# SADPR/1D-Burgers-Equation-ROMs

Hardware: AMD Instinct MI355X
Metric: batched Newton-steps/sec over mu-sweep (sample-Newton-steps/s, FOM N=1024) (higher is better)
Workload: dtype f64

## Files before the change

### 1d-burgers-equation-roms_amd/csrc/fom.hip

```cpp
#include <hip/hip_runtime.h>
#include <stdint.h>
#include <type_traits>

#include "../../include/burgers_hip.h"
#include "abi_common.hpp"
#include "fom_device.hpp"
#include "fom_wide.hpp"

namespace bg {
thread_local int tls_last_hip_error = 0;
}

namespace {

using namespace bg;

struct FomArgs {
    const double* x;
    const double* u0;
    const double* mu1;
    const double* mu2;
    double* hist;
    int32_t* iters;
    int32_t* flags;
    double dt, E, tol2;
    int N, B, nsteps, max_it, supg;
    double* errs;
};

constexpr int WAVES_PER_WG = 4;

template <int R>
__device__ __forceinline__ void load_rows(const double* __restrict__ src, int N, int row0, bool full,
                                          double (&u)[R], double pad = 0.0)
{
#pragma unroll
    for (int j = 0; j < R; ++j) u[j] = (full || row0 + j < N) ? src[row0 + j] : pad;
}

template <int R>
__device__ __forceinline__ void store_rows(double* __restrict__ dst, int N, int row0, bool full,
                                           const double (&u)[R])
{
#pragma unroll
    for (int j = 0; j < R; ++j)
        if (full || row0 + j < N) dst[row0 + j] = u[j];
}

template <int R, bool FULL, bool UNI, bool TRACE, bool PARK, class Topo>
__device__ __forceinline__ void fom_sample(const FomArgs& a, Topo& tp, int s, WidePark<PARK ? R : 1>* park)
{
    static_assert(UNI || !PARK, "only the uniform assembly reads g and hfs through accessors");
    const int N = a.N, t = tp.g, row0 = t * R;
    const double h = (a.x[N - 1] - a.x[0]) / (double)(N - 1);
    const MeshConst c = make_mesh_const(h, a.dt, a.E, a.supg);
    const double mu1 = a.mu1[s], mu2 = a.mu2[s];

    double hfs[PARK ? 1 : R], fdt[R], u[R], g[PARK ? 1 : R];
    ElemGeom<UNI ? 0 : R> gm;
    if constexpr (PARK) {
        double hf[R];
        forcing_setup<R>(a.x, N, row0, mu2, c.h, a.dt, hf, fdt);
#pragma unroll
        for (int j = 0; j < R; ++j) park->hfs[j][t] = hf[j];
    } else if constexpr (UNI) {
        forcing_setup<R>(a.x, N, row0, mu2, c.h, a.dt, hfs, fdt);
    } else {
        geom_setup<R>(a.x, N, row0, a.dt, a.E, gm);
        forcing_setup_general<R>(a.x, N, row0, mu2, a.dt, hfs, fdt);
    }
    auto g_put = [&](int j, double v) { if constexpr (PARK) park->g[j][t] = v; else g[j] = v; };
    auto g_at = [&](int j) { if constexpr (PARK) return park->g[j][t]; else return g[j]; };
    auto hf_at = [&](int j) { if constexpr (PARK) return park->hfs[j][t]; else return hfs[j]; };

    double* hist = a.hist + (size_t)s * (size_t)(a.nsteps + 1) * (size_t)N;
    load_rows<R>(a.u0 + (size_t)s * N, N, row0, FULL, u);
    store_rows<R>(hist, N, row0, FULL, u);

    int flags = 0;
    for (int step = 0; step < a.nsteps; ++step) {
        if constexpr (UNI) mass_rhs<R, FULL>(tp, c, N, u, fdt, g_put);
        else mass_rhs_general<R>(tp, gm, N, u, fdt, g);
        int k = 0;
        bool more;
        do {
            double lo[R], di[R], up[R], rhs[R];
            if constexpr (UNI) assemble<R, FULL>(tp, c, N, mu1, u, g_at, hf_at, lo, di, up, rhs);
            else assemble_general<R>(tp, gm, a.dt, c.kap, N, mu1, u, g, hfs, lo, di, up, rhs);
            tp.template solve<R>(lo, di, up, rhs);
            double nd = 0.0, nu = 0.0;
#pragma unroll
            for (int j = 0; j < R; ++j) {
                u[j] += rhs[j];
                nd = __builtin_fma(rhs[j], rhs[j], nd);
                nu = __builtin_fma(u[j], u[j], nu);
            }
            tp.sum2(nd, nu, nd, nu);
            if constexpr (TRACE) {
                if (tp.first()) a.errs[((size_t)s * a.nsteps + step) * a.max_it + k] = sqrt(nd) / sqrt(nu);
            }
            ++k;
            more = (nd > a.tol2 * nu) && (k < a.max_it);
            flags |= uniform_nonfinite(nd, nu) ? BG_FLAG_NONFINITE : 0;
        } while (more);
        if (k >= a.max_it) flags |= BG_FLAG_HIT_CAP;
        store_rows<R>(hist + (size_t)(step + 1) * N, N, row0, FULL, u);
        if (tp.first()) a.iters[(size_t)s * a.nsteps + step] = k;
    }
    if (tp.first()) a.flags[s] = flags;
}

struct AsmArgs {
    const double *x, *uk, *un, *mu1, *mu2;
    double *lo, *di, *up, *rhs;
    double dt, E;
    int N, B, supg;
};

template <int R, bool FULL, bool UNI, class Topo>
__device__ __forceinline__ void assemble_sample(const AsmArgs& a, Topo& tp, int s)
{
    const int N = a.N, row0 = tp.g * R;
    const double h = (a.x[N - 1] - a.x[0]) / (double)(N - 1);
    const MeshConst c = make_mesh_const(h, a.dt, a.E, a.supg);
    double hfs[R], fdt[R], u[R], un[R], g[R], lo[R], di[R], up[R], rhs[R];
    load_rows<R>(a.un + (size_t)s * N, N, row0, FULL, un);
    load_rows<R>(a.uk + (size_t)s * N, N, row0, FULL, u);
    if constexpr (UNI) {
        forcing_setup<R>(a.x, N, row0, a.mu2[s], c.h, a.dt, hfs, fdt);
        auto g_put = [&](int j, double v) { g[j] = v; };
        auto g_at = [&](int j) { return g[j]; };
        auto hf_at = [&](int j) { return hfs[j]; };
        mass_rhs<R, FULL>(tp, c, N, un, fdt, g_put);
        assemble<R, FULL>(tp, c, N, a.mu1[s], u, g_at, hf_at, lo, di, up, rhs);
    } else {
        ElemGeom<R> gm;
        geom_setup<R>(a.x, N, row0, a.dt, a.E, gm);
        forcing_setup_general<R>(a.x, N, row0, a.mu2[s], a.dt, hfs, fdt);
        mass_rhs_general<R>(tp, gm, N, un, fdt, g);
        assemble_general<R>(tp, gm, a.dt, c.kap, N, a.mu1[s], u, g, hfs, lo, di, up, rhs);
    }
    store_rows<R>(a.lo + (size_t)s * N, N, row0, FULL, lo);
    store_rows<R>(a.di + (size_t)s * N, N, row0, FULL, di);
    store_rows<R>(a.up + (size_t)s * N, N, row0, FULL, up);
    store_rows<R>(a.rhs + (size_t)s * N, N, row0, FULL, rhs);
}

struct SolveArgs {
    const double *lo, *di, *up, *rhs;
    double* sol;
    int N, B;
};

template <int R, class Topo>
__device__ __forceinline__ void solve_sample(const SolveArgs& a, Topo& tp, int s)
{
    const int N = a.N, row0 = tp.g * R;
    double lo[R], di[R], up[R], rhs[R];
    const size_t off = (size_t)s * N;
    load_rows<R>(a.lo + off, N, row0, false, lo);
    load_rows<R>(a.di + off, N, row0, false, di, 1.0);
    load_rows<R>(a.up + off, N, row0, false, up);
    load_rows<R>(a.rhs + off, N, row0, false, rhs);
    tp.template solve<R>(lo, di, up, rhs);
    store_rows<R>(a.sol + off, N, row0, false, rhs);
}

template <int R, bool FULL, bool UNI = true, bool TRACE = false>
__global__ __launch_bounds__(64 * WAVES_PER_WG, 1) void fom_fused_kernel(FomArgs a)
{
    const int s = blockIdx.x * WAVES_PER_WG + (int)(threadIdx.x >> 6);
    if (s >= a.B) return;
    WaveTopo tp{lane_id()};
    fom_sample<R, FULL, UNI, TRACE, false>(a, tp, s, nullptr);
}

template <int R, bool FULL, bool UNI = true>
__global__ __launch_bounds__(64 * WAVES_PER_WG, 1) void fom_assemble_kernel(AsmArgs a)
{
    const int s = blockIdx.x * WAVES_PER_WG + (int)(threadIdx.x >> 6);
    if (s >= a.B) return;
    WaveTopo tp{lane_id()};
    assemble_sample<R, FULL, UNI>(a, tp, s);
}

template <int R>
__global__ __launch_bounds__(64 * WAVES_PER_WG, 1) void tridiag_solve_kernel(SolveArgs a)
{
    const int s = blockIdx.x * WAVES_PER_WG + (int)(threadIdx.x >> 6);
    if (s >= a.B) return;
    WaveTopo tp{lane_id()};
    solve_sample<R>(a, tp, s);
}

template <int R, bool UNI>
__global__ __launch_bounds__(WIDE_THREADS, 1) void fom_wide_kernel(FomArgs a)
{
    constexpr bool PARK = UNI && R >= 32;
    __shared__ WideLds lds;
    __shared__ WidePark<PARK ? R : 1> park;
    wide_init(lds, threadIdx.x);
    WgTopo tp{lds, (int)threadIdx.x, 0};
    fom_sample<R, false, UNI, false, PARK>(a, tp, blockIdx.x, &park);
}

template <int R, bool UNI>
__global__ __launch_bounds__(WIDE_THREADS, 1) void fom_assemble_wide_kernel(AsmArgs a)
{
    __shared__ WideLds lds;
    wide_init(lds, threadIdx.x);
    WgTopo tp{lds, (int)threadIdx.x, 0};
    assemble_sample<R, false, UNI>(a, tp, blockIdx.x);
}

template <int R>
__global__ __launch_bounds__(WIDE_THREADS, 1) void tridiag_solve_wide_kernel(SolveArgs a)
{
    __shared__ WideLds lds;
    wide_init(lds, threadIdx.x);
    WgTopo tp{lds, (int)threadIdx.x, 0};
    solve_sample<R>(a, tp, blockIdx.x);
}

__global__ __launch_bounds__(256) void transpose_kernel(const double* __restrict__ in,
                                                        double* __restrict__ out, int nb, int rows, int cols)
{
    __shared__ double tile[32][33];
    const int c0 = blockIdx.x * 32, r0 = blockIdx.y * 32;
    const int tx = threadIdx.x & 31, ty = threadIdx.x >> 5;
    for (int b = blockIdx.z; b < nb; b += gridDim.z) {
        const size_t base = (size_t)b * rows * cols;
#pragma unroll
        for (int k = 0; k < 32; k += 8) {
            int r = r0 + ty + k, cc = c0 + tx;
            if (r < rows && cc < cols) tile[ty + k][tx] = in[base + (size_t)r * cols + cc];
        }
        __syncthreads();
#pragma unroll
        for (int k = 0; k < 32; k += 8) {
            int cc = c0 + ty + k, r = r0 + tx;
            if (r < rows && cc < cols) out[base + (size_t)cc * rows + r] = tile[tx][ty + k];
        }
        __syncthreads();
    }
}

constexpr int kWaveMaxN = 64 * 24, kWideMaxN = WIDE_THREADS * 32;

template <typename F>
int dispatch_wide(int N, F&& f)
{
    return dispatch_rows<WIDE_THREADS, 2, 4, 8, 12, 16, 24, 32>(N, f);
}

template <typename F>
int dispatch_r(int N, F&& f)
{
    return dispatch_rows<64, 1, 2, 3, 4, 5, 6, 8, 9, 10, 12, 16, 24>(N, f);
}

int fom_args(FomArgs& a, bool traced, int N, int B, int nsteps, const double* x, const double* u0, const double* mu1,
             const double* mu2, double dt, double E, double tol, int max_it, int supg, double* hist, int32_t* iters,
             int32_t* flags, double* errs)
{
    if (N < 2 || B < 0 || nsteps < 0 || max_it < 1 || !(dt > 0.0)) return BG_ERR_BAD_ARG;
    if (traced && N > kWaveMaxN) return BG_ERR_UNSUPPORTED_N;
    if (B == 0) return BG_OK;
    if (!x || !u0 || !mu1 || !mu2 || !hist || !flags || (traced && !errs) || (nsteps > 0 && !iters)) return BG_ERR_BAD_ARG;
    a.x = x; a.u0 = u0; a.mu1 = mu1; a.mu2 = mu2; a.hist = hist; a.iters = iters; a.flags = flags; a.errs = errs;
    a.dt = dt; a.E = E; a.tol2 = tol * tol;
    a.N = N; a.B = B; a.nsteps = nsteps; a.max_it = max_it; a.supg = supg & BG_OPT_SUPG;
    return BG_OK;
}

}

extern "C" {

int bg_abi_version(void) { return BG_ABI_VERSION; }

int bg_last_hip_error(void) { return bg::tls_last_hip_error; }

int bg_fom_max_n(void) { return kWideMaxN; }

const char* bg_strerror(int code)
{
    switch (code) {
        case BG_OK: return "ok";
        case BG_ERR_BAD_ARG: return "bad argument";
        case BG_ERR_UNSUPPORTED_N: return "N not supported by the fused kernels (2 <= N <= 8192)";
        case BG_ERR_NONUNIFORM: return "mesh is not uniform";
        case BG_ERR_LAUNCH: return "kernel launch failed (see bg_last_hip_error)";
        case BG_ERR_UNSUPPORTED_R: return "reduced dimension not supported";
        case BG_ERR_PROJECTION: return "unknown projection";
        case BG_ERR_WORKSPACE: return "workspace too small";
        default: return "unknown error";
    }
}

int bg_fom_run(int N, int B, int nsteps, const double* x, const double* u0, const double* mu1,
               const double* mu2, double dt, double E, double tol, int max_it, int supg, double* hist,
               int32_t* iters, int32_t* flags, void* stream)
{
    FomArgs a;
    const int err = fom_args(a, false, N, B, nsteps, x, u0, mu1, mu2, dt, E, tol, max_it, supg, hist, iters, flags, nullptr);
    if (err != BG_OK || B == 0) return err;
    const bool nonuniform = (supg & BG_OPT_NONUNIFORM) != 0;
    const dim3 grid((B + WAVES_PER_WG - 1) / WAVES_PER_WG), block(64 * WAVES_PER_WG);
    hipStream_t st = (hipStream_t)stream;
    const bool both = N <= kWaveMaxN && N > 64 && !nonuniform;
    const bool wide = N > kWaveMaxN || (both && (supg & BG_OPT_FOM_WIDE) && !(supg & BG_OPT_FOM_WAVE));
    if (wide)
        return dispatch_wide(N, [&](auto rc) {
            constexpr int R = decltype(rc)::value;
            if constexpr (R >= 8) {
                if (nonuniform) {
                    hipLaunchKernelGGL((fom_wide_kernel<R, false>), dim3(B), dim3(WIDE_THREADS), 0, st, a);
                    return check_launch();
                }
            }
            hipLaunchKernelGGL((fom_wide_kernel<R, true>), dim3(B), dim3(WIDE_THREADS), 0, st, a);
            return check_launch();
        });
    return dispatch_r(N, [&](auto rc) {
        constexpr int R = decltype(rc)::value;
        if (nonuniform)
            hipLaunchKernelGGL((fom_fused_kernel<R, false, false>), grid, block, 0, st, a);
        else if (N == 64 * R)
            hipLaunchKernelGGL((fom_fused_kernel<R, true>), grid, block, 0, st, a);
        else
            hipLaunchKernelGGL((fom_fused_kernel<R, false>), grid, block, 0, st, a);
        return check_launch();
    });
}

int bg_fom_run_traced(int N, int B, int nsteps, const double* x, const double* u0, const double* mu1, const double* mu2,
                      double dt, double E, double tol, int max_it, int supg, double* hist, int32_t* iters, int32_t* flags,
                      double* errs, void* stream)
{
    FomArgs a;
    const int err = fom_args(a, true, N, B, nsteps, x, u0, mu1, mu2, dt, E, tol, max_it, supg, hist, iters, flags, errs);
    if (err != BG_OK || B == 0) return err;
    const bool nonuniform = (supg & BG_OPT_NONUNIFORM) != 0;
    const dim3 grid((B + WAVES_PER_WG - 1) / WAVES_PER_WG), block(64 * WAVES_PER_WG);
    hipStream_t st = (hipStream_t)stream;
    return dispatch_r(N, [&](auto rc) {
        constexpr int R = decltype(rc)::value;
        if (nonuniform)
            hipLaunchKernelGGL((fom_fused_kernel<R, false, false, true>), grid, block, 0, st, a);
        else
            hipLaunchKernelGGL((fom_fused_kernel<R, false, true, true>), grid, block, 0, st, a);
        return check_launch();
    });
}

int bg_fom_assemble(int N, int B, const double* x, const double* uk, const double* un, const double* mu1,
                    const double* mu2, double dt, double E, int supg, double* lo, double* di, double* up,
                    double* rhs, void* stream)
{
    if (N < 2 || B < 0 || !(dt > 0.0)) return BG_ERR_BAD_ARG;
    if (B == 0) return BG_OK;
    if (!x || !uk || !un || !mu1 || !mu2 || !lo || !di || !up || !rhs) return BG_ERR_BAD_ARG;
    AsmArgs a;
    a.x = x; a.uk = uk; a.un = un; a.mu1 = mu1; a.mu2 = mu2; a.lo = lo; a.di = di; a.up = up; a.rhs = rhs;
    a.dt = dt; a.E = E; a.N = N; a.B = B; a.supg = supg & BG_OPT_SUPG;
    const bool nonuniform = (supg & BG_OPT_NONUNIFORM) != 0;
    const dim3 grid((B + WAVES_PER_WG - 1) / WAVES_PER_WG), block(64 * WAVES_PER_WG);
    hipStream_t st = (hipStream_t)stream;
    if (N > kWaveMaxN)
        return dispatch_wide(N, [&](auto rc) {
            constexpr int R = decltype(rc)::value;
            if (nonuniform)
                hipLaunchKernelGGL((fom_assemble_wide_kernel<R, false>), dim3(B), dim3(WIDE_THREADS), 0, st, a);
            else
                hipLaunchKernelGGL((fom_assemble_wide_kernel<R, true>), dim3(B), dim3(WIDE_THREADS), 0, st, a);
            return check_launch();
        });
    return dispatch_r(N, [&](auto rc) {
        constexpr int R = decltype(rc)::value;
        if (nonuniform)
            hipLaunchKernelGGL((fom_assemble_kernel<R, false, false>), grid, block, 0, st, a);
        else if (N == 64 * R)
            hipLaunchKernelGGL((fom_assemble_kernel<R, true>), grid, block, 0, st, a);
        else
            hipLaunchKernelGGL((fom_assemble_kernel<R, false>), grid, block, 0, st, a);
        return check_launch();
    });
}

int bg_tridiag_solve(int N, int B, const double* lo, const double* di, const double* up, const double* rhs,
                     double* sol, void* stream)
{
    if (N < 1 || B < 0) return BG_ERR_BAD_ARG;
    if (B == 0) return BG_OK;
    if (!lo || !di || !up || !rhs || !sol) return BG_ERR_BAD_ARG;
    SolveArgs a{lo, di, up, rhs, sol, N, B};
    const dim3 grid((B + WAVES_PER_WG - 1) / WAVES_PER_WG), block(64 * WAVES_PER_WG);
    hipStream_t st = (hipStream_t)stream;
    if (N > kWaveMaxN)
        return dispatch_wide(N, [&](auto rc) {
            constexpr int R = decltype(rc)::value;
            hipLaunchKernelGGL((tridiag_solve_wide_kernel<R>), dim3(B), dim3(WIDE_THREADS), 0, st, a);
            return check_launch();
        });
    return dispatch_r(N, [&](auto rc) {
        constexpr int R = decltype(rc)::value;
        hipLaunchKernelGGL((tridiag_solve_kernel<R>), grid, block, 0, st, a);
        return check_launch();
    });
}

int bg_transpose_batched(int B, int rows, int cols, const double* in, double* out, void* stream)
{
    if (B < 0 || rows < 0 || cols < 0) return BG_ERR_BAD_ARG;
    if (B == 0 || rows == 0 || cols == 0) return BG_OK;
    if (!in || !out) return BG_ERR_BAD_ARG;
    const dim3 grid((cols + 31) / 32, (rows + 31) / 32, B < 65535 ? B : 65535), block(256);
    hipLaunchKernelGGL(transpose_kernel, grid, block, 0, (hipStream_t)stream, in, out, B, rows, cols);
    return check_launch();
}

}
```

### 1d-burgers-equation-roms_amd/csrc/fom_device.hpp

```cpp
#pragma once
#include "wave_ops.hpp"

#ifndef BG_RCP
#define BG_RCP rcp1
#endif

#ifndef BG_PCR_EARLY_EXIT
#define BG_PCR_EARLY_EXIT 1
#endif

namespace bg {

constexpr double GP_A = 0.78867513459481287;
constexpr double GP_B = 0.21132486540518713;

struct MeshConst {
    double h;
    double aoff;
    double dd2;
    double dd1;
    double dt6;
    double kap;
    double h6;
};

__device__ __forceinline__ MeshConst make_mesh_const(double h, double dt, double E, int supg)
{
    MeshConst c;
    c.h = h;
    double eh = dt * E / h;
    c.aoff = h / 6.0 - eh;
    c.dd1 = h / 3.0 + eh;
    c.dd2 = 2.0 * c.dd1;
    c.dt6 = dt / 6.0;
    c.kap = supg ? 0.25 * dt : 0.0;
    c.h6 = h / 6.0;
    return c;
}

template <int R>
__device__ __forceinline__ void forcing_setup(const double* __restrict__ x, int N, int row0, double mu2,
                                              double h, double dt, double (&hfs)[R], double (&fdt)[R])
{
    double frPrev = 0.0;
    {
        int e = row0 - 1;
        if (e >= 0 && e < N - 1) {
            double xl = x[e], xr = x[e + 1];
            double f1 = 0.02 * exp(mu2 * (GP_A * xl + GP_B * xr));
            double f2 = 0.02 * exp(mu2 * (GP_B * xl + GP_A * xr));
            frPrev = (f1 * GP_B + f2 * GP_A) * (0.5 * h);
        }
    }
#pragma unroll
    for (int j = 0; j < R; ++j) {
        int e = row0 + j;
        double fl = 0.0, fr = 0.0, fs = 0.0;
        if (e < N - 1) {
            double xl = x[e], xr = x[e + 1];
            double f1 = 0.02 * exp(mu2 * (GP_A * xl + GP_B * xr));
            double f2 = 0.02 * exp(mu2 * (GP_B * xl + GP_A * xr));
            fl = (f1 * GP_A + f2 * GP_B) * (0.5 * h);
            fr = (f1 * GP_B + f2 * GP_A) * (0.5 * h);
            fs = f1 + f2;
        }
        hfs[j] = h * fs;
        fdt[j] = (e < N) ? dt * (frPrev + fl) : 0.0;
        frPrev = fr;
    }
}

template <int R, bool FULL, class Topo, typename GStore>
__device__ __forceinline__ void mass_rhs(Topo& tp, const MeshConst& c, int N, const double (&u)[R],
                                         const double (&fdt)[R], GStore&& gstore)
{
    double uL, uR;
    tp.halo(u[0], u[R - 1], uL, uR);
#pragma unroll
    for (int j = 0; j < R; ++j) {
        const double um = (j == 0) ? uL : u[j - 1];
        const double up = (j == R - 1) ? uR : u[j + 1];
        const int i = tp.g * R + j;
        double m = __builtin_fma(4.0, u[j], um) + up;
        if (FULL ? (j == R - 1) : true) {
            const bool is_last = FULL ? tp.last() : (i == N - 1);
            m = is_last ? __builtin_fma(2.0, u[j], um) : m;
        }
        double v = __builtin_fma(c.h6, m, fdt[j]);
        gstore(j, (!FULL && i >= N) ? 0.0 : v);
    }
    tp.halo_done();
}

template <int R>
__device__ __forceinline__ void supg_terms(const double (&mx)[R], const double (&t)[R], double (&se)[R])
{
    constexpr int G = R / 4 * 4;
#pragma unroll
    for (int j = 0; j < G; j += 4) {
        const double p01 = mx[j] * mx[j + 1], p23 = mx[j + 2] * mx[j + 3];
        const double r = BG_RCP(p01 * p23);
        const double r01 = r * p23, r23 = r * p01;
        se[j] = t[j] * (r01 * mx[j + 1]);
        se[j + 1] = t[j + 1] * (r01 * mx[j]);
        se[j + 2] = t[j + 2] * (r23 * mx[j + 3]);
        se[j + 3] = t[j + 3] * (r23 * mx[j + 2]);
    }
#pragma unroll
    for (int j = G; j < R; ++j) se[j] = t[j] * BG_RCP(mx[j]);
}

template <int R, typename HF>
__device__ __forceinline__ void assemble_p1(const MeshConst& c, const double (&u)[R], double uL, double uR,
                                            HF&& hf, double (&lo)[R], double (&up)[R], double (&se)[R])
{
    double mx[R], t[R];
#pragma unroll
    for (int j = 0; j < R; ++j) {
        const double ur = (j == R - 1) ? uR : u[j + 1];
        const double w = u[j] + ur;
        const double dif = ur - u[j];
        up[j] = __builtin_fma(c.dt6, w + u[j], c.aoff);
        if (j + 1 < R) lo[j + 1] = __builtin_fma(-c.dt6, w + ur, c.aoff);
        mx[j] = fmax(fabs(w), 2.0e-10);
        t[j] = __builtin_fma(w, dif, -hf(j));
    }
    supg_terms<R>(mx, t, se);
    lo[0] = __builtin_fma(-c.dt6, __builtin_fma(2.0, u[0], uL), c.aoff);
}

template <int R, bool FULL, typename GF>
__device__ __forceinline__ void assemble_p2(const MeshConst& c, int N, int row0, bool first, bool last_lane,
                                            double mu1, const double (&u)[R], double uL, double uR, double seL,
                                            GF&& g, const double (&se)[R], double (&lo)[R],
                                            double (&di)[R], double (&up)[R], double (&rhs)[R])
{
#pragma unroll
    for (int j = 0; j < R; ++j) {
        const double um = (j == 0) ? uL : u[j - 1];
        const double ur = (j == R - 1) ? uR : u[j + 1];
        const double sm = (j == 0) ? seL : se[j - 1];
        const int i = row0 + j;
        double d = __builtin_fma(c.dt6, um - ur, c.dd2);
        double b = __builtin_fma(-c.kap, sm, g(j));
        double bb = __builtin_fma(c.kap, se[j], b);
        double l = lo[j], p = up[j];
        const bool is_last = FULL ? (j == R - 1 && last_lane) : (i == N - 1);
        if (FULL ? (j == R - 1) : true) {
            double dl = __builtin_fma(c.dt6, __builtin_fma(2.0, u[j], um), c.dd1);
            d = is_last ? dl : d;
            p = is_last ? 0.0 : p;
            bb = is_last ? b : bb;
        }
        if (!FULL) {
            const bool pad = i >= N;
            d = pad ? 1.0 : d;
            p = pad ? 0.0 : p;
            l = pad ? 0.0 : l;
            bb = pad ? 0.0 : bb;
        }
        if (j == 0) {
            d = first ? 1.0 : d;
            p = first ? 0.0 : p;
            l = first ? 0.0 : l;
            bb = first ? mu1 : bb;
        }
        double r = __builtin_fma(-l, um, bb);
        r = __builtin_fma(-d, u[j], r);
        r = __builtin_fma(-p, ur, r);
        lo[j] = l; di[j] = d; up[j] = p; rhs[j] = r;
    }
}

template <int R, bool FULL, class Topo, typename GF, typename HF>
__device__ __forceinline__ void assemble(Topo& tp, const MeshConst& c, int N, double mu1, const double (&u)[R], GF&& g,
                                         HF&& hf, double (&lo)[R], double (&di)[R], double (&up)[R], double (&rhs)[R])
{
    double uL, uR, se[R];
    tp.halo(u[0], u[R - 1], uL, uR);
    assemble_p1<R>(c, u, uL, uR, hf, lo, up, se);
    const double seL = tp.below_se(se[R - 1]);
    assemble_p2<R, FULL>(c, N, tp.g * R, tp.first(), tp.last(), mu1, u, uL, uR, seL, g, se, lo, di, up, rhs);
}

template <int R>
struct ElemGeom {
    double h6[R + 1];
    double eh[R + 1];
};

template <int R>
__device__ __forceinline__ void geom_setup(const double* __restrict__ x, int N, int row0, double dt, double E,
                                           ElemGeom<R>& gm)
{
#pragma unroll
    for (int j = 0; j <= R; ++j) {
        const int e = row0 + j - 1;
        double h = 1.0;
        if (e >= 0 && e < N - 1) h = x[e + 1] - x[e];
        gm.h6[j] = (e >= 0 && e < N - 1) ? h / 6.0 : 0.0;
        gm.eh[j] = (e >= 0 && e < N - 1) ? dt * E / h : 0.0;
    }
}

template <int R>
__device__ __forceinline__ void forcing_setup_general(const double* __restrict__ x, int N, int row0, double mu2,
                                                      double dt, double (&hfs)[R], double (&fdt)[R])
{
    double frPrev = 0.0;
#pragma unroll
    for (int j = -1; j < R; ++j) {
        const int e = row0 + j;
        double fl = 0.0, fr = 0.0, hf = 0.0;
        if (e >= 0 && e < N - 1) {
            const double xl = x[e], xr = x[e + 1], h = xr - xl;
            const double f1 = 0.02 * exp(mu2 * (GP_A * xl + GP_B * xr));
            const double f2 = 0.02 * exp(mu2 * (GP_B * xl + GP_A * xr));
            fl = (f1 * GP_A + f2 * GP_B) * (0.5 * h);
            fr = (f1 * GP_B + f2 * GP_A) * (0.5 * h);
            hf = h * (f1 + f2);
        }
        if (j >= 0) {
            hfs[j] = hf;
            fdt[j] = (e < N) ? dt * (frPrev + fl) : 0.0;
        }
        frPrev = fr;
    }
}

template <int R, class Topo>
__device__ __forceinline__ void mass_rhs_general(Topo& tp, const ElemGeom<R>& gm, int N, const double (&u)[R],
                                                 const double (&fdt)[R], double (&g)[R])
{
    double uL, uR;
    tp.halo(u[0], u[R - 1], uL, uR);
#pragma unroll
    for (int j = 0; j < R; ++j) {
        const double um = (j == 0) ? uL : u[j - 1];
        const double up = (j == R - 1) ? uR : u[j + 1];
        const int i = tp.g * R + j;
        double v = gm.h6[j] * __builtin_fma(2.0, u[j], um);
        v = __builtin_fma(gm.h6[j + 1], __builtin_fma(2.0, u[j], up), v);
        g[j] = (i >= N) ? 0.0 : v + fdt[j];
    }
    tp.halo_done();
}

template <int R>
__device__ __forceinline__ void assemble_general_p1(const ElemGeom<R>& gm, double dt, const double (&u)[R], double uL,
                                                    double uR, const double (&hfs)[R], double (&lo)[R],
                                                    double (&up)[R], double (&se)[R])
{
    const double dt6 = dt / 6.0;
    double mx[R], t[R];
#pragma unroll
    for (int j = 0; j < R; ++j) {
        const double ur = (j == R - 1) ? uR : u[j + 1];
        const double w = u[j] + ur;
        const double dif = ur - u[j];
        const double aoff = gm.h6[j + 1] - gm.eh[j + 1];
        up[j] = __builtin_fma(dt6, w + u[j], aoff);
        if (j + 1 < R) lo[j + 1] = __builtin_fma(-dt6, w + ur, aoff);
        mx[j] = fmax(fabs(w), 2.0e-10);
        t[j] = __builtin_fma(w, dif, -hfs[j]);
    }
    supg_terms<R>(mx, t, se);
    lo[0] = __builtin_fma(-dt6, __builtin_fma(2.0, u[0], uL), gm.h6[0] - gm.eh[0]);
}

template <int R>
__device__ __forceinline__ void assemble_general_p2(const ElemGeom<R>& gm, double dt, double kap, int N, int row0,
                                                    bool first, double mu1, const double (&u)[R], double uL,
                                                    double uR, double seL, const double (&g)[R],
                                                    const double (&se)[R], double (&lo)[R], double (&di)[R],
                                                    double (&up)[R], double (&rhs)[R])
{
    const double dt6 = dt / 6.0;
#pragma unroll
    for (int j = 0; j < R; ++j) {
        const double um = (j == 0) ? uL : u[j - 1];
        const double ur = (j == R - 1) ? uR : u[j + 1];
        const double sm = (j == 0) ? seL : se[j - 1];
        const int i = row0 + j;
        const double ddl = __builtin_fma(2.0, gm.h6[j], gm.eh[j]);
        const double ddr = __builtin_fma(2.0, gm.h6[j + 1], gm.eh[j + 1]);
        double d = __builtin_fma(dt6, um - ur, ddl + ddr);
        double b = __builtin_fma(-kap, sm, g[j]);
        double bb = __builtin_fma(kap, se[j], b);
        double l = lo[j], p = up[j];
        const bool is_last = (i == N - 1);
        const double dl = __builtin_fma(dt6, __builtin_fma(2.0, u[j], um), ddl);
        d = is_last ? dl : d;
        p = is_last ? 0.0 : p;
        bb = is_last ? b : bb;
        const bool pad = i >= N;
        d = pad ? 1.0 : d;
        p = pad ? 0.0 : p;
        l = pad ? 0.0 : l;
        bb = pad ? 0.0 : bb;
        if (j == 0) {
            d = first ? 1.0 : d;
            p = first ? 0.0 : p;
            l = first ? 0.0 : l;
            bb = first ? mu1 : bb;
        }
        double r = __builtin_fma(-l, um, bb);
        r = __builtin_fma(-d, u[j], r);
        r = __builtin_fma(-p, ur, r);
        lo[j] = l; di[j] = d; up[j] = p; rhs[j] = r;
    }
}

template <int R, class Topo>
__device__ __forceinline__ void assemble_general(Topo& tp, const ElemGeom<R>& gm, double dt, double kap, int N,
                                                 double mu1, const double (&u)[R], const double (&g)[R],
                                                 const double (&hfs)[R], double (&lo)[R], double (&di)[R],
                                                 double (&up)[R], double (&rhs)[R])
{
    double uL, uR, se[R];
    tp.halo(u[0], u[R - 1], uL, uR);
    assemble_general_p1<R>(gm, dt, u, uL, uR, hfs, lo, up, se);
    const double seL = tp.below_se(se[R - 1]);
    assemble_general_p2<R>(gm, dt, kap, N, tp.g * R, tp.first(), mu1, u, uL, uR, seL, g, se, lo, di, up, rhs);
}

template <int CTRL_DN, int CTRL_UP, int REPS>
__device__ __forceinline__ double pcr_step_rhs(double A, double C, double D)
{
    const double Dm = dpp_shift<CTRL_DN, REPS>(D), Dp = dpp_shift<CTRL_UP, REPS>(D);
    return __builtin_fma(-Dp, C, __builtin_fma(-Dm, A, D));
}

template <int CTRL_DN, int CTRL_UP, int REPS, bool LAST>
__device__ __forceinline__ void pcr_step(double& A, double& C, double& D)
{
    const double Cm = dpp_shift<CTRL_DN, REPS>(C), Ap = dpp_shift<CTRL_UP, REPS>(A);
    double Bn = __builtin_fma(-Cm, A, 1.0);
    Bn = __builtin_fma(-Ap, C, Bn);
    const double Dn = pcr_step_rhs<CTRL_DN, CTRL_UP, REPS>(A, C, D);
    const double rb = BG_RCP(Bn);
    D = Dn * rb;
    if (!LAST) {
        const double Am = dpp_shift<CTRL_DN, REPS>(A), Cp = dpp_shift<CTRL_UP, REPS>(C);
        A = -(Am * A) * rb;
        C = -(Cp * C) * rb;
    }
}

template <int R>
__device__ __forceinline__ double wang_reduce(double (&lo)[R], double (&di)[R], const double (&up)[R],
                                              double (&rhs)[R], double (&gs)[R])
{
    static_assert(R > 1, "R == 1 has no interior rows");
    double dp = di[0];
    di[0] = BG_RCP(dp);
#pragma unroll
    for (int j = 1; j < R; ++j) {
        const double m = lo[j] * di[j - 1];
        dp = __builtin_fma(-m, up[j - 1], di[j]);
        di[j] = BG_RCP(dp);
        rhs[j] = __builtin_fma(-m, rhs[j - 1], rhs[j]);
        lo[j] = -m * lo[j - 1];
    }
    gs[R - 2] = up[R - 2];
#pragma unroll
    for (int j = R - 3; j >= 0; --j) {
        const double t = up[j] * di[j + 1];
        rhs[j] = __builtin_fma(-t, rhs[j + 1], rhs[j]);
        lo[j] = __builtin_fma(-t, lo[j + 1], lo[j]);
        gs[j] = -t * gs[j + 1];
    }
    return dp;
}

template <int R>
__device__ __forceinline__ void wang_interface(const double (&lo)[R], const double (&up)[R], const double (&rhs)[R],
                                               double dp, double F0, double G0, double R0, double& A, double& C,
                                               double& D)
{
    const double ul = up[R - 1];
    const double B = __builtin_fma(-ul, F0, dp);
    const double rb = BG_RCP(B);
    A = lo[R - 1] * rb;
    C = -(ul * G0) * rb;
    D = __builtin_fma(-ul, R0, rhs[R - 1]) * rb;
}

template <int R>
__device__ __forceinline__ void wang_finish(const double (&lo)[R], const double (&di)[R], double (&rhs)[R],
                                            const double (&gs)[R], double X, double XL)
{
#pragma unroll
    for (int j = 0; j < R - 1; ++j) {
        double v = __builtin_fma(-lo[j], XL, rhs[j]);
        v = __builtin_fma(-gs[j], X, v);
        rhs[j] = v * di[j];
    }
    rhs[R - 1] = X;
}

__device__ __forceinline__ double pcr64(double A, double C, double D)
{
    const int lane = lane_id();
    pcr_step<0x138, 0x130, 1, false>(A, C, D);
    pcr_step<0x138, 0x130, 2, false>(A, C, D);
    {
        const int src = ((4 * (lane & 15) + (lane >> 4)) << 2);
        A = from_lane_rot(A, src); C = from_lane_rot(C, src); D = from_lane_rot(D, src);
    }
    pcr_step<0x111, 0x101, 1, false>(A, C, D);
#if BG_PCR_EARLY_EXIT
    constexpr double tau = 0x1p-31;
    const bool coupled = !(__builtin_fabs(A) <= tau && __builtin_fabs(C) <= tau);
    const bool full = __builtin_amdgcn_ballot_w64(coupled) != 0;
    const double D4 = D;
    D = pcr_step_rhs<0x112, 0x102, 1>(A, C, D4);
    if (__builtin_expect(full, 0)) {
        D = D4;
        pcr_step<0x112, 0x102, 1, false>(A, C, D);
        pcr_step<0x114, 0x104, 1, false>(A, C, D);
        pcr_step<0x118, 0x108, 1, true>(A, C, D);
    }
#else
    pcr_step<0x112, 0x102, 1, false>(A, C, D);
    pcr_step<0x114, 0x104, 1, false>(A, C, D);
    pcr_step<0x118, 0x108, 1, true>(A, C, D);
#endif
    return from_lane_rot(D, (16 * (lane & 3) + (lane >> 2)) << 2);
}

template <int R>
__device__ __forceinline__ void tridiag_solve(double (&lo)[R], double (&di)[R], const double (&up)[R],
                                              double (&rhs)[R])
{
    if constexpr (R == 1) {
        const double rb = BG_RCP(di[0]);
        rhs[0] = pcr64(lo[0] * rb, up[0] * rb, rhs[0] * rb);
    } else {
        double gs[R];
        const double dp = wang_reduce<R>(lo, di, up, rhs, gs);
        const double F0 = from_lane_above(lo[0] * di[0]);
        const double G0 = from_lane_above(gs[0] * di[0]);
        const double R0 = from_lane_above(rhs[0] * di[0]);
        double A, C, D;
        wang_interface<R>(lo, up, rhs, dp, F0, G0, R0, A, C, D);
        const double X = pcr64(A, C, D);
        wang_finish<R>(lo, di, rhs, gs, X, from_lane_below(X));
    }
}

}
```

### 1d-burgers-equation-roms_amd/csrc/fom_wide.hpp

```cpp
#pragma once
#include "fom_device.hpp"

namespace bg {

constexpr int WIDE_WAVES = 4;
constexpr int WIDE_THREADS = 64 * WIDE_WAVES;
constexpr int WIDE_PAD = 2;
constexpr int WIDE_LEN = WIDE_THREADS + 2 * WIDE_PAD;

struct WideLds {
    double ufirst[WIDE_LEN], ulast[WIDE_LEN];
    double se[WIDE_LEN];
    double fgr[3][WIDE_LEN];
    double pcr[2][3][WIDE_LEN];
    double x[WIDE_LEN];
    double nrm[2][WIDE_WAVES];
};

__device__ __forceinline__ void wide_init(WideLds& s, int tid)
{
    double* p = reinterpret_cast<double*>(&s);
    for (int i = tid; i < (int)(sizeof(WideLds) / sizeof(double)); i += WIDE_THREADS) p[i] = 0.0;
    __syncthreads();
}

template <int R>
struct WidePark {
    double g[R][WIDE_THREADS];
    double hfs[R][WIDE_THREADS];
};

template <int S>
__device__ __forceinline__ void wide_pcr_step(const double (&buf)[3][WIDE_LEN], int e, double& A, double& C, double& D)
{
    const int m = e + WIDE_PAD - S, p = e + WIDE_PAD + S;
    const double Am = buf[0][m], Cm = buf[1][m], Dm = buf[2][m];
    const double Ap = buf[0][p], Cp = buf[1][p], Dp = buf[2][p];
    double Bn = __builtin_fma(-Cm, A, 1.0);
    Bn = __builtin_fma(-Ap, C, Bn);
    double Dn = __builtin_fma(-Dm, A, D);
    Dn = __builtin_fma(-Dp, C, Dn);
    const double rb = BG_RCP(Bn);
    D = Dn * rb;
    A = -(Am * A) * rb;
    C = -(Cp * C) * rb;
}

template <int R>
__device__ __forceinline__ void wide_tridiag_solve(WideLds& s, int g, double (&lo)[R], double (&di)[R],
                                                   const double (&up)[R], double (&rhs)[R])
{
    double gs[R];
    const double dp = wang_reduce<R>(lo, di, up, rhs, gs);
    s.fgr[0][g + WIDE_PAD] = lo[0] * di[0];
    s.fgr[1][g + WIDE_PAD] = gs[0] * di[0];
    s.fgr[2][g + WIDE_PAD] = rhs[0] * di[0];
    __syncthreads();
    double A, C, D;
    wang_interface<R>(lo, up, rhs, dp, s.fgr[0][g + WIDE_PAD + 1], s.fgr[1][g + WIDE_PAD + 1],
                      s.fgr[2][g + WIDE_PAD + 1], A, C, D);
    s.pcr[0][0][g + WIDE_PAD] = A;
    s.pcr[0][1][g + WIDE_PAD] = C;
    s.pcr[0][2][g + WIDE_PAD] = D;
    __syncthreads();
    const int e = (g & 63) * WIDE_WAVES + (g >> 6);
    A = s.pcr[0][0][e + WIDE_PAD]; C = s.pcr[0][1][e + WIDE_PAD]; D = s.pcr[0][2][e + WIDE_PAD];
    wide_pcr_step<1>(s.pcr[0], e, A, C, D);
    s.pcr[1][0][e + WIDE_PAD] = A;
    s.pcr[1][1][e + WIDE_PAD] = C;
    s.pcr[1][2][e + WIDE_PAD] = D;
    __syncthreads();
    wide_pcr_step<2>(s.pcr[1], e, A, C, D);
    s.x[e + WIDE_PAD] = pcr64(A, C, D);
    __syncthreads();
    wang_finish<R>(lo, di, rhs, gs, s.x[g + WIDE_PAD], s.x[g + WIDE_PAD - 1]);
}

__device__ __forceinline__ void wide_sum2(WideLds& s, int g, double a, double b, double& sa, double& sb)
{
    wave_sum2(a, b, a, b);
    if ((g & 63) == 0) { s.nrm[0][g >> 6] = a; s.nrm[1][g >> 6] = b; }
    __syncthreads();
    sa = (s.nrm[0][0] + s.nrm[0][1]) + (s.nrm[0][2] + s.nrm[0][3]);
    sb = (s.nrm[1][0] + s.nrm[1][1]) + (s.nrm[1][2] + s.nrm[1][3]);
}

__device__ __forceinline__ double wave_max(double v)
{
    v = fmax(v, dpp_mov<0x111>(v));
    v = fmax(v, dpp_mov<0x112>(v));
    v = fmax(v, dpp_mov<0x114>(v));
    v = fmax(v, dpp_mov<0x118>(v));
    v = fmax(v, dpp_mov<0x142, 0xA>(v));
    v = fmax(v, dpp_mov<0x143, 0xC>(v));
    int lo = __builtin_amdgcn_readlane(__double2loint(v), 63);
    int hi = __builtin_amdgcn_readlane(__double2hiint(v), 63);
    return __hiloint2double(hi, lo);
}

__device__ __forceinline__ double wave_max_nan(double v, bool nan)
{
    const double m = wave_max(v);
    return __builtin_amdgcn_ballot_w64(nan) ? __builtin_nan("") : m;
}

struct WaveTopo {
    int g;
    __device__ __forceinline__ bool first() const { return g == 0; }
    __device__ __forceinline__ bool last() const { return g == 63; }
    __device__ __forceinline__ void halo(double first, double last, double& uL, double& uR)
    {
        uL = from_lane_below(last);
        uR = from_lane_above(first);
    }
    __device__ __forceinline__ void halo_done() {}
    __device__ __forceinline__ double below_se(double v) { return from_lane_below(v); }
    __device__ __forceinline__ double below(double v) { return from_lane_below(v); }
    __device__ __forceinline__ double above(double v) { return from_lane_above(v); }
    __device__ __forceinline__ double gmax(double v) { return wave_max(v); }
    __device__ __forceinline__ double gmax_nan(double v, bool nan) { return wave_max_nan(v, nan); }
    __device__ __forceinline__ void sum2(double a, double b, double& sa, double& sb) { wave_sum2(a, b, sa, sb); }
    template <int R>
    __device__ __forceinline__ void solve(double (&lo)[R], double (&di)[R], const double (&up)[R], double (&rhs)[R])
    {
        tridiag_solve<R>(lo, di, up, rhs);
    }
};

struct WgTopo {
    WideLds& s;
    int g;
    int par;
    __device__ __forceinline__ bool first() const { return g == 0; }
    __device__ __forceinline__ bool last() const { return g == WIDE_THREADS - 1; }
    __device__ __forceinline__ void halo(double first, double last, double& uL, double& uR)
    {
        s.ufirst[g + WIDE_PAD] = first;
        s.ulast[g + WIDE_PAD] = last;
        __syncthreads();
        uL = s.ulast[g + WIDE_PAD - 1];
        uR = s.ufirst[g + WIDE_PAD + 1];
    }
    __device__ __forceinline__ void halo_done() { __syncthreads(); }
    __device__ __forceinline__ double below_se(double v)
    {
        s.se[g + WIDE_PAD] = v;
        __syncthreads();
        return s.se[g + WIDE_PAD - 1];
    }
    __device__ __forceinline__ double shift(double v, int d)
    {
        double* buf = par ? s.ulast : s.ufirst;
        par ^= 1;
        buf[g + WIDE_PAD] = v;
        __syncthreads();
        return buf[g + WIDE_PAD + d];
    }
    __device__ __forceinline__ double below(double v) { return shift(v, -1); }
    __device__ __forceinline__ double above(double v) { return shift(v, +1); }
    __device__ __forceinline__ double gmax(double v)
    {
        v = wave_max(v);
        double* buf = s.nrm[par];
        par ^= 1;
        if ((g & 63) == 0) buf[g >> 6] = v;
        __syncthreads();
        return fmax(fmax(buf[0], buf[1]), fmax(buf[2], buf[3]));
    }
    __device__ __forceinline__ double gmax_nan(double v, bool nan)
    {
        v = wave_max_nan(v, nan);
        double* buf = s.nrm[par];
        par ^= 1;
        if ((g & 63) == 0) buf[g >> 6] = v;
        __syncthreads();
        const double b0 = buf[0], b1 = buf[1], b2 = buf[2], b3 = buf[3];
        const double m = fmax(fmax(b0, b1), fmax(b2, b3));
        return ((b0 != b0) | (b1 != b1) | (b2 != b2) | (b3 != b3)) ? __builtin_nan("") : m;
    }
    __device__ __forceinline__ void sum2(double a, double b, double& sa, double& sb) { wide_sum2(s, g, a, b, sa, sb); }
    template <int R>
    __device__ __forceinline__ void solve(double (&lo)[R], double (&di)[R], const double (&up)[R], double (&rhs)[R])
    {
        wide_tridiag_solve<R>(s, g, lo, di, up, rhs);
    }
};

}
```

### 1d-burgers-equation-roms_amd/csrc/wave_ops.hpp

```cpp
#pragma once
#include <hip/hip_runtime.h>

#include "../../include/burgers_hip.h"

namespace bg {

constexpr int WAVE = 64;

__device__ __forceinline__ int lane_id() { return (int)(threadIdx.x & 63u); }

template <int CTRL, int ROW_MASK = 0xF, bool BOUND_ZERO = true>
__device__ __forceinline__ double dpp_mov(double v, double old = 0.0)
{
    int lo = __double2loint(v), hi = __double2hiint(v);
    int olo = __double2loint(old), ohi = __double2hiint(old);
    lo = __builtin_amdgcn_update_dpp(olo, lo, CTRL, ROW_MASK, 0xF, BOUND_ZERO);
    hi = __builtin_amdgcn_update_dpp(ohi, hi, CTRL, ROW_MASK, 0xF, BOUND_ZERO);
    return __hiloint2double(hi, lo);
}

__device__ __forceinline__ double from_lane_below(double v) { return dpp_mov<0x138>(v); }
__device__ __forceinline__ double from_lane_above(double v) { return dpp_mov<0x130>(v); }

__device__ __forceinline__ double from_lane_rot(double v, int src_lane_times4)
{
    int lo = __double2loint(v), hi = __double2hiint(v);
    lo = __builtin_amdgcn_ds_bpermute(src_lane_times4, lo);
    hi = __builtin_amdgcn_ds_bpermute(src_lane_times4, hi);
    return __hiloint2double(hi, lo);
}

__device__ __forceinline__ double wave_sum(double v)
{
    v += dpp_mov<0x111>(v);
    v += dpp_mov<0x112>(v);
    v += dpp_mov<0x114>(v);
    v += dpp_mov<0x118>(v);
    v += dpp_mov<0x142, 0xA>(v);
    v += dpp_mov<0x143, 0xC>(v);
    int lo = __builtin_amdgcn_readlane(__double2loint(v), 63);
    int hi = __builtin_amdgcn_readlane(__double2hiint(v), 63);
    return __hiloint2double(hi, lo);
}

__device__ __forceinline__ double rcp(double d)
{
    double r = __builtin_amdgcn_rcp(d);
    double e = __builtin_fma(-d, r, 1.0);
    r = __builtin_fma(r, e, r);
    e = __builtin_fma(-d, r, 1.0);
    r = __builtin_fma(r, e, r);
    return r;
}

__device__ __forceinline__ double rcp1(double d)
{
    double r = __builtin_amdgcn_rcp(d);
    double e = __builtin_fma(-d, r, 1.0);
    return __builtin_fma(r, e, r);
}

template <int CTRL, int REPS>
__device__ __forceinline__ double dpp_shift(double v)
{
#pragma unroll
    for (int i = 0; i < REPS; ++i) v = dpp_mov<CTRL>(v);
    return v;
}

__device__ __forceinline__ void wave_sum2(double a, double b, double& sa, double& sb)
{
    auto l = __builtin_amdgcn_permlane32_swap((unsigned)__double2loint(a), (unsigned)__double2loint(b), false, false);
    auto h = __builtin_amdgcn_permlane32_swap((unsigned)__double2hiint(a), (unsigned)__double2hiint(b), false, false);
    double v = __hiloint2double((int)h[0], (int)l[0]) + __hiloint2double((int)h[1], (int)l[1]);
    v += dpp_mov<0x111>(v);
    v += dpp_mov<0x112>(v);
    v += dpp_mov<0x114>(v);
    v += dpp_mov<0x118>(v);
    v += dpp_mov<0x142, 0xA>(v);
    sa = __hiloint2double(__builtin_amdgcn_readlane(__double2hiint(v), 31),
                          __builtin_amdgcn_readlane(__double2loint(v), 31));
    sb = __hiloint2double(__builtin_amdgcn_readlane(__double2hiint(v), 63),
                          __builtin_amdgcn_readlane(__double2loint(v), 63));
}

__device__ __forceinline__ double sel(bool c, double a, double b) { return c ? a : b; }

constexpr unsigned F64_EXP_HI = 0x7ff00000u;
__device__ __forceinline__ unsigned uniform_exponent_bits(double v)
{
    unsigned hi = (unsigned)__builtin_amdgcn_readfirstlane(__double2hiint(v));
    asm("" : "+s"(hi));
    return hi & F64_EXP_HI;
}
__device__ __forceinline__ bool uniform_nonfinite(double v) { return uniform_exponent_bits(v) == F64_EXP_HI; }
__device__ __forceinline__ bool uniform_nonfinite(double a, double b)
{
    const unsigned ea = uniform_exponent_bits(a), eb = uniform_exponent_bits(b);
    return (ea > eb ? ea : eb) == F64_EXP_HI;
}

template <int CTRL>
__device__ __forceinline__ float dpp_f32(float v)
{
    return __builtin_bit_cast(float, __builtin_amdgcn_update_dpp(0, __builtin_bit_cast(int, v), CTRL, 0xF, 0xF, true));
}

__device__ __forceinline__ float swap16_add(float a, float b)
{
    const auto t = __builtin_amdgcn_permlane16_swap(__builtin_bit_cast(unsigned, a), __builtin_bit_cast(unsigned, b), false, false);
    return __builtin_bit_cast(float, (unsigned)t[0]) + __builtin_bit_cast(float, (unsigned)t[1]);
}
__device__ __forceinline__ float swap32_add(float a, float b)
{
    const auto t = __builtin_amdgcn_permlane32_swap(__builtin_bit_cast(unsigned, a), __builtin_bit_cast(unsigned, b), false, false);
    return __builtin_bit_cast(float, (unsigned)t[0]) + __builtin_bit_cast(float, (unsigned)t[1]);
}

__device__ __forceinline__ void mlp_activate(int kind, float alpha, float v, float& av, float& d)
{
    av = v; d = 1.0f;
    if (kind == BG_ACT_ELU) {
        const float e = alpha * expf(v);
        av = v > 0.0f ? v : e - alpha;
        d = v > 0.0f ? 1.0f : e;
    } else if (kind == BG_ACT_RELU) {
        av = v > 0.0f ? v : 0.0f;
        d = v > 0.0f ? 1.0f : 0.0f;
    } else if (kind == BG_ACT_TANH) {
        av = tanhf(v);
        d = 1.0f - av * av;
    }
}

#ifdef BG_PHASE_CLOCK
constexpr bool kPhaseClock = true;
#else
constexpr bool kPhaseClock = false;
#endif

template <bool ON, int SLOTS>
struct PhaseClock {
    long long cyc[SLOTS] = {};
    long long real0, tick;
    int passes = 0;
    __device__ __forceinline__ PhaseClock()
        : real0((long long)__builtin_amdgcn_s_memrealtime()), tick((long long)__builtin_amdgcn_s_memtime()) {}
    __device__ __forceinline__ void lap(int i)
    {
        const long long now = (long long)__builtin_amdgcn_s_memtime();
        cyc[i] += now - tick;
        tick = now;
    }
    __device__ __forceinline__ void pass() { ++passes; }
    __device__ __forceinline__ void store(int32_t* iters_row, int nsteps) const
    {
        if (nsteps < SLOTS + 3) return;
        long long total = (long long)__builtin_amdgcn_s_memtime() - tick;
#pragma unroll
        for (int i = 0; i < SLOTS; ++i) {
            iters_row[i] = (int)(cyc[i] >> 10);
            total += cyc[i];
        }
        iters_row[SLOTS] = passes;
        iters_row[SLOTS + 1] = (int)(total >> 10);
        iters_row[SLOTS + 2] = (int)(((long long)__builtin_amdgcn_s_memrealtime() - real0) >> 10);
    }
};
template <int SLOTS>
struct PhaseClock<false, SLOTS> {
    __device__ __forceinline__ void lap(int) const {}
    __device__ __forceinline__ void pass() const {}
    __device__ __forceinline__ void store(int32_t*, int) const {}
};

}
```

Before: 577.7 million.

## Rotate Newton loop to overlap next assembly head with convergence reduction

Splits assembly into a head (halo exchange plus per-row p1 terms) and a tail, then rotates the Newton loop so the next iteration's head runs right after the update. For the wave topology it interleaves the DPP cross-lane reduction rounds of the convergence norms with chunks of the p1 assembly, hiding reduction latency behind independent arithmetic. This adds live registers (hlo, hup, hse) and redundant head work after the last iteration, which may raise register pressure.

```diff
diff --git a/1d-burgers-equation-roms_amd/csrc/fom.hip b/1d-burgers-equation-roms_amd/csrc/fom.hip
--- a/1d-burgers-equation-roms_amd/csrc/fom.hip
+++ b/1d-burgers-equation-roms_amd/csrc/fom.hip
@@ -77,6 +77,17 @@
     load_rows<R>(a.u0 + (size_t)s * N, N, row0, FULL, u);
     store_rows<R>(hist, N, row0, FULL, u);
 
+    constexpr bool ROT = BG_PICARD_ROTATE && Topo::rotates_picard;
+    static_assert(!ROT || !PARK, "the parked form belongs to the workgroup topology");
+    double huL, huR, hse[ROT ? R : 1], hlo[ROT ? R : 1], hup[ROT ? R : 1];
+    auto head = [&]() {
+        if constexpr (ROT) {
+            if constexpr (UNI) assemble_head<R>(tp, c, u, hf_at, huL, huR, hse, hlo, hup);
+            else assemble_general_head<R>(tp, gm, a.dt, u, hfs, huL, huR, hse, hlo, hup);
+        }
+    };
+    head();
+
     int flags = 0;
     for (int step = 0; step < a.nsteps; ++step) {
         if constexpr (UNI) mass_rhs<R, FULL>(tp, c, N, u, fdt, g_put);
@@ -85,8 +96,15 @@
         bool more;
         do {
             double lo[R], di[R], up[R], rhs[R];
-            if constexpr (UNI) assemble<R, FULL>(tp, c, N, mu1, u, g_at, hf_at, lo, di, up, rhs);
-            else assemble_general<R>(tp, gm, a.dt, c.kap, N, mu1, u, g, hfs, lo, di, up, rhs);
+            if constexpr (ROT) {
+#pragma unroll
+                for (int j = 0; j < R; ++j) { lo[j] = hlo[j]; up[j] = hup[j]; }
+                if constexpr (UNI) assemble_tail<R, FULL>(tp, c, N, mu1, u, g_at, huL, huR, hse, lo, di, up, rhs);
+                else assemble_general_tail<R>(tp, gm, a.dt, c.kap, N, mu1, u, g, huL, huR, hse, lo, di, up, rhs);
+            } else {
+                if constexpr (UNI) assemble<R, FULL>(tp, c, N, mu1, u, g_at, hf_at, lo, di, up, rhs);
+                else assemble_general<R>(tp, gm, a.dt, c.kap, N, mu1, u, g, hfs, lo, di, up, rhs);
+            }
             tp.template solve<R>(lo, di, up, rhs);
             double nd = 0.0, nu = 0.0;
 #pragma unroll
@@ -95,7 +113,25 @@
                 nd = __builtin_fma(rhs[j], rhs[j], nd);
                 nu = __builtin_fma(u[j], u[j], nu);
             }
-            tp.sum2(nd, nu, nd, nu);
+            if constexpr (ROT && UNI) {
+                WaveSum2 ws;
+                tp.halo(u[0], u[R - 1], huL, huR);
+                ws.start(nd, nu);
+                auto weave = [&](auto kc) {
+                    constexpr int K = decltype(kc)::value, J0 = 4 * K, J1 = J0 + 4 < R ? J0 + 4 : R;
+                    if constexpr (K < 5) ws.template round<K>();
+                    if constexpr (J0 < R) assemble_p1_rows<R, J0, J1>(c, u, huR, hf_at, hlo, hup, hse);
+                };
+                static_assert(R <= 24, "six chunks");
+                weave(std::integral_constant<int, 0>{}); weave(std::integral_constant<int, 1>{});
+                weave(std::integral_constant<int, 2>{}); weave(std::integral_constant<int, 3>{});
+                weave(std::integral_constant<int, 4>{}); weave(std::integral_constant<int, 5>{});
+                hlo[0] = __builtin_fma(-c.dt6, __builtin_fma(2.0, u[0], huL), c.aoff);
+                ws.finish(nd, nu);
+            } else {
+                head();
+                tp.sum2(nd, nu, nd, nu);
+            }
             if constexpr (TRACE) {
                 if (tp.first()) a.errs[((size_t)s * a.nsteps + step) * a.max_it + k] = sqrt(nd) / sqrt(nu);
             }
diff --git a/1d-burgers-equation-roms_amd/csrc/fom_device.hpp b/1d-burgers-equation-roms_amd/csrc/fom_device.hpp
--- a/1d-burgers-equation-roms_amd/csrc/fom_device.hpp
+++ b/1d-burgers-equation-roms_amd/csrc/fom_device.hpp
@@ -7,6 +7,10 @@
 
 #ifndef BG_PCR_EARLY_EXIT
 #define BG_PCR_EARLY_EXIT 1
+#endif
+
+#ifndef BG_PICARD_ROTATE
+#define BG_PICARD_ROTATE 1
 #endif
 
 namespace bg {
@@ -127,6 +131,37 @@
     }
     supg_terms<R>(mx, t, se);
     lo[0] = __builtin_fma(-c.dt6, __builtin_fma(2.0, u[0], uL), c.aoff);
+}
+
+template <int R, int J0, int J1, typename HF>
+__device__ __forceinline__ void assemble_p1_rows(const MeshConst& c, const double (&u)[R], double uR, HF&& hf,
+                                                 double (&lo)[R], double (&up)[R], double (&se)[R])
+{
+    constexpr int G = R / 4 * 4;
+    static_assert(J0 % 4 == 0 && J0 < J1 && J1 <= R && (J0 < G ? J1 == J0 + 4 : J1 == R), "one supg group or the remainder");
+    double mx[4], t[4];
+#pragma unroll
+    for (int j = J0; j < J1; ++j) {
+        const double ur = (j == R - 1) ? uR : u[j + 1];
+        const double w = u[j] + ur;
+        const double dif = ur - u[j];
+        up[j] = __builtin_fma(c.dt6, w + u[j], c.aoff);
+        if (j + 1 < R) lo[j + 1] = __builtin_fma(-c.dt6, w + ur, c.aoff);
+        mx[j - J0] = fmax(fabs(w), 2.0e-10);
+        t[j - J0] = __builtin_fma(w, dif, -hf(j));
+    }
+    if constexpr (J0 < G) {
+        const double p01 = mx[0] * mx[1], p23 = mx[2] * mx[3];
+        const double r = BG_RCP(p01 * p23);
+        const double r01 = r * p23, r23 = r * p01;
+        se[J0] = t[0] * (r01 * mx[1]);
+        se[J0 + 1] = t[1] * (r01 * mx[0]);
+        se[J0 + 2] = t[2] * (r23 * mx[3]);
+        se[J0 + 3] = t[3] * (r23 * mx[2]);
+    } else {
+#pragma unroll
+        for (int j = J0; j < J1; ++j) se[j] = t[j - J0] * BG_RCP(mx[j - J0]);
+    }
 }
 
 template <int R, bool FULL, typename GF>
@@ -170,6 +205,23 @@
         r = __builtin_fma(-p, ur, r);
         lo[j] = l; di[j] = d; up[j] = p; rhs[j] = r;
     }
+}
+
+template <int R, class Topo, typename HF>
+__device__ __forceinline__ void assemble_head(Topo& tp, const MeshConst& c, const double (&u)[R], HF&& hf, double& uL,
+                                              double& uR, double (&se)[R], double (&lo)[R], double (&up)[R])
+{
+    tp.halo(u[0], u[R - 1], uL, uR);
+    assemble_p1<R>(c, u, uL, uR, hf, lo, up, se);
+}
+
+template <int R, bool FULL, class Topo, typename GF>
+__device__ __forceinline__ void assemble_tail(Topo& tp, const MeshConst& c, int N, double mu1, const double (&u)[R],
+                                              GF&& g, double uL, double uR, const double (&se)[R], double (&lo)[R],
+                                              double (&di)[R], double (&up)[R], double (&rhs)[R])
+{
+    const double seL = tp.below_se(se[R - 1]);
+    assemble_p2<R, FULL>(c, N, tp.g * R, tp.first(), tp.last(), mu1, u, uL, uR, seL, g, se, lo, di, up, rhs);
 }
 
 template <int R, bool FULL, class Topo, typename GF, typename HF>
@@ -312,6 +364,25 @@
 }
 
 template <int R, class Topo>
+__device__ __forceinline__ void assemble_general_head(Topo& tp, const ElemGeom<R>& gm, double dt, const double (&u)[R],
+                                                      const double (&hfs)[R], double& uL, double& uR, double (&se)[R],
+                                                      double (&lo)[R], double (&up)[R])
+{
+    tp.halo(u[0], u[R - 1], uL, uR);
+    assemble_general_p1<R>(gm, dt, u, uL, uR, hfs, lo, up, se);
+}
+
+template <int R, class Topo>
+__device__ __forceinline__ void assemble_general_tail(Topo& tp, const ElemGeom<R>& gm, double dt, double kap, int N,
+                                                      double mu1, const double (&u)[R], const double (&g)[R], double uL,
+                                                      double uR, const double (&se)[R], double (&lo)[R],
+                                                      double (&di)[R], double (&up)[R], double (&rhs)[R])
+{
+    const double seL = tp.below_se(se[R - 1]);
+    assemble_general_p2<R>(gm, dt, kap, N, tp.g * R, tp.first(), mu1, u, uL, uR, seL, g, se, lo, di, up, rhs);
+}
+
+template <int R, class Topo>
 __device__ __forceinline__ void assemble_general(Topo& tp, const ElemGeom<R>& gm, double dt, double kap, int N,
                                                  double mu1, const double (&u)[R], const double (&g)[R],
                                                  const double (&hfs)[R], double (&lo)[R], double (&di)[R],
diff --git a/1d-burgers-equation-roms_amd/csrc/fom_wide.hpp b/1d-burgers-equation-roms_amd/csrc/fom_wide.hpp
--- a/1d-burgers-equation-roms_amd/csrc/fom_wide.hpp
+++ b/1d-burgers-equation-roms_amd/csrc/fom_wide.hpp
@@ -105,6 +105,7 @@
 }
 
 struct WaveTopo {
+    static constexpr bool rotates_picard = true;
     int g;
     __device__ __forceinline__ bool first() const { return g == 0; }
     __device__ __forceinline__ bool last() const { return g == 63; }
@@ -128,6 +129,7 @@
 };
 
 struct WgTopo {
+    static constexpr bool rotates_picard = false;
     WideLds& s;
     int g;
     int par;
diff --git a/1d-burgers-equation-roms_amd/csrc/wave_ops.hpp b/1d-burgers-equation-roms_amd/csrc/wave_ops.hpp
--- a/1d-burgers-equation-roms_amd/csrc/wave_ops.hpp
+++ b/1d-burgers-equation-roms_amd/csrc/wave_ops.hpp
@@ -84,6 +84,32 @@
                           __builtin_amdgcn_readlane(__double2loint(v), 63));
 }
 
+struct WaveSum2 {
+    double v;
+    __device__ __forceinline__ void start(double a, double b)
+    {
+        auto l = __builtin_amdgcn_permlane32_swap((unsigned)__double2loint(a), (unsigned)__double2loint(b), false, false);
+        auto h = __builtin_amdgcn_permlane32_swap((unsigned)__double2hiint(a), (unsigned)__double2hiint(b), false, false);
+        v = __hiloint2double((int)h[0], (int)l[0]) + __hiloint2double((int)h[1], (int)l[1]);
+    }
+    template <int I>
+    __device__ __forceinline__ void round()
+    {
+        if constexpr (I == 0) v += dpp_mov<0x111>(v);
+        if constexpr (I == 1) v += dpp_mov<0x112>(v);
+        if constexpr (I == 2) v += dpp_mov<0x114>(v);
+        if constexpr (I == 3) v += dpp_mov<0x118>(v);
+        if constexpr (I == 4) v += dpp_mov<0x142, 0xA>(v);
+    }
+    __device__ __forceinline__ void finish(double& sa, double& sb) const
+    {
+        sa = __hiloint2double(__builtin_amdgcn_readlane(__double2hiint(v), 31),
+                              __builtin_amdgcn_readlane(__double2loint(v), 31));
+        sb = __hiloint2double(__builtin_amdgcn_readlane(__double2hiint(v), 63),
+                              __builtin_amdgcn_readlane(__double2loint(v), 63));
+    }
+};
+
 __device__ __forceinline__ double sel(bool c, double a, double b) { return c ? a : b; }
 
 constexpr unsigned F64_EXP_HI = 0x7ff00000u;
```

Result: faster. 592.4 million, median of 6 (+2.6%).
